# chaofengc/FeMaSR

Hardware: AMD Instinct MI355X
Metric: SR output megapixels/sec at x4 (128->512) (higher is better)
Workload: dtype f32 (1x1 convs / nn.Linear: every fp32 operand split EXACTLY into three bf16 terms, six partial products, fp32 accumulation on the bf16 matrix pipe - closer to fp64 than the fp32 fmaf chain, bit-identical to the CPU oracle)

## Files before the change

femasr_amd/_lib.py:

```python
import ctypes
import os

_HERE = os.path.dirname(os.path.abspath(__file__))
SO_PATH = os.path.join(_HERE, 'csrc', 'libfemasr_hip.so')

c_int, c_i64, c_f32 = ctypes.c_int, ctypes.c_int64, ctypes.c_float
vp, szt = ctypes.c_void_p, ctypes.c_size_t


class FemasrError(RuntimeError):
    pass


MAX_CODEBOOKS = 3


class Config(ctypes.Structure):
    _fields_ = ([(n, ctypes.c_int32) for n in ('in_channel', 'gt_resolution', 'lq_stage', 'scale_factor', 'use_quantize',
                                               'use_residual', 'n_codebooks')] +
                [(n, ctypes.c_int32 * MAX_CODEBOOKS) for n in ('codebook_scale', 'n_e', 'e_dim')] +
                [('device', ctypes.c_int32)])


class ConvArgs(ctypes.Structure):
# ... 107 lines not shown
    'femasr_niqe_plane_offsets': (c_int, [c_int, c_int, c_int, c_int, ctypes.POINTER(szt * 4)]),
    'femasr_niqe_features': (c_int, [vp, vp, c_int, c_int, c_int, c_int, vp, vp, vp, vp, c_int, vp, vp, c_int, vp, vp, vp, szt]),
    'femasr_color_fix_workspace_bytes': (c_int, [c_int, c_int, c_int, c_int, c_int, c_int, ctypes.POINTER(szt)]),
    'femasr_color_fix': (c_int, [vp, vp, vp, c_int, c_int, c_int, c_int, c_int, c_int, c_int, vp, vp, c_int, vp, vp, c_int, vp, vp, szt]),
    'femasr_color_fix_u8': (c_int, [vp, vp, vp, c_int, c_int, c_int, c_int, c_int, c_int, c_int, vp, vp, c_int, vp, vp, c_int, vp, vp, szt]),
    'femasr_dihedral_expand': (c_int, [vp, vp, c_int, c_int, c_int, c_int, vp, vp]),
    'femasr_dihedral_expand_u8': (c_int, [vp, vp, c_int, c_int, c_int, vp, vp]),
    'femasr_dihedral_merge': (c_int, [vp, vp, vp, c_int, c_int, c_int, c_int, vp]),
    'femasr_dihedral_merge_u8': (c_int, [vp, vp, vp, c_int, c_int, c_int, vp]),
    'femasr_png_filter_rgb8': (c_int, [vp, vp, c_int, c_int, c_int, c_int, vp]),
    'femasr_png_filter_u8': (c_int, [vp, vp, c_int, c_int, c_int, c_int, c_int, vp]),
    'femasr_channels_split_u8': (c_int, [vp, vp, c_int, c_int, c_int, c_int, vp, vp]),
    'femasr_channels_merge_u8': (c_int, [vp, vp, vp, vp, c_int, c_int, c_int, c_int, vp, vp, c_int, vp, vp, c_int, vp]),
    'femasr_clock_probe': (c_int, [vp, c_int, vp]),
    'femasr_clock_probe_entries': (c_int, []),
}
DEBUG_SIGNATURES = {
    'femasr_debug_set_wino_limits': (c_int, [vp, c_int, c_int]),
    'femasr_debug_mfma_bf16': (c_int, [vp, vp, vp, vp, c_int, vp]),
    'femasr_gemm_force_config': (c_int, [c_int]),
    'femasr_conv_small_launch_blocks': (c_int, [c_int]),
    'femasr_debug_conv_variant_name': (c_int, [ctypes.POINTER(ConvArgs), ctypes.c_char_p, c_int]),
    'femasr_debug_weight_image_bytes': (c_int, [vp, c_int, ctypes.POINTER(szt)]),
}

_lib = None


def load():
    global _lib
    if _lib is not None:
        return _lib
    if not os.path.exists(SO_PATH):
        raise FemasrError(
            f'{SO_PATH} not found: the HIP extension is not built. Run `python femasr_amd/csrc/build.py` '
            '(needs hipcc; cross-compiles gfx950 without a GPU). There is no CPU fallback.')
    lib = ctypes.CDLL(SO_PATH)
    lib.femasr_version.restype = c_int
    if lib.femasr_version() != ABI_VERSION:
        raise FemasrError(f'{SO_PATH} reports ABI version {lib.femasr_version()}, this binding is written for {ABI_VERSION} '
                          '(femasr_conv_args layout): rebuild with `python femasr_amd/csrc/build.py --force`')
    for name, (res, args) in list(SIGNATURES.items()) + list(DEBUG_SIGNATURES.items()):
        fn = getattr(lib, name)
        fn.restype = res
        fn.argtypes = args
    _lib = lib
# ... 12 lines not shown
```

femasr_amd/csrc/build.py:

```python
import os
import subprocess
import sys

HERE = os.path.dirname(os.path.abspath(__file__))
SOURCES = ['kernels_conv.hip', 'kernels_gemm.hip', 'kernels_gemm_bf16.hip', 'kernels_gemm_f16.hip', 'kernels_vq.hip', 'kernels_norm.hip', 'kernels_attn.hip', 'kernels_layout.hip', 'kernels_probe.hip', 'conv_forms.hip', 'kernels_wino.hip', 'kernels_wino_up2.hip', 'kernels_conv_bf16.hip', 'kernels_conv_f16.hip', 'model.hip', 'lpips.hip', 'psnr_ssim.hip', 'niqe.hip', 'colorfix.hip', 'ensemble.hip', 'png_filter.hip', 'channels.hip']
HEADERS = ['common.h', 'conv_common.h', 'halo_mma.h', 'wino_common.h', 'gemm_common.h', 'detmath.h', 'pixel.h', '../../include/femasr_hip.h', '../../include/femasr_hip_debug.h']
SO = os.path.join(HERE, 'libfemasr_hip.so')
FLAGS = ['--offload-arch=gfx950', '-O3', '-std=c++17', '-fPIC', '-ffp-contract=off',
         '-fhip-fp32-correctly-rounded-divide-sqrt', '-Wno-unused-result']


def _stale(target, deps):
    if not os.path.exists(target):
        return True
    t = os.path.getmtime(target)
    return any(os.path.getmtime(d) > t for d in deps)


def build(force=False, verbose=True, gate='fail'):
    hipcc = os.environ.get('HIPCC', '/opt/rocm/bin/hipcc')
    hdrs = [os.path.join(HERE, h) for h in HEADERS]
    objs, jobs = [], []
    for src in SOURCES:
        s = os.path.join(HERE, src)
        o = os.path.join(HERE, src.replace('.hip', '.o'))
        if force or _stale(o, [s] + hdrs):
            cmd = [hipcc] + FLAGS + ['-c', s, '-o', o]
            if verbose:
                print(' '.join(cmd), flush=True)
# ... 33 lines not shown
```

femasr_amd/csrc/common.h:

```cpp
#pragma once
#include <hip/hip_runtime.h>
#include <stdint.h>
#include <stddef.h>
#include "../../include/femasr_hip_debug.h"

int femasr_set_error(int code, const char *fmt, ...);
#define FEMASR_CHECK_HIP(expr)                                                            \
    do {                                                                                  \
        hipError_t _e = (expr);                                                           \
        if (_e != hipSuccess)                                                             \
            return femasr_set_error(FEMASR_ERR_HIP, "%s failed: %s (%s:%d)", #expr,       \
                                    hipGetErrorString(_e), __FILE__, __LINE__);           \
    } while (0)
#define FEMASR_REQUIRE(cond, ...)                                                         \
    do {                                                                                  \
        if (!(cond)) return femasr_set_error(FEMASR_ERR_INVALID, __VA_ARGS__);            \
    } while (0)

inline int femasr_allow_dynamic_lds(const void *kern, unsigned long long *devs, size_t bytes)
{
    int dev = 0;
    FEMASR_CHECK_HIP(hipGetDevice(&dev));
    if (dev < 0 || dev >= 64 || !((__atomic_load_n(devs, __ATOMIC_ACQUIRE) >> dev) & 1ull)) {
        FEMASR_CHECK_HIP(hipFuncSetAttribute(kern, hipFuncAttributeMaxDynamicSharedMemorySize, (int)bytes));
        if (dev >= 0 && dev < 64) __atomic_fetch_or(devs, 1ull << dev, __ATOMIC_RELEASE);
    }
    return FEMASR_OK;
}
#define FEMASR_CHECK(expr) do { const int _rc = (expr); if (_rc != FEMASR_OK) return _rc; } while (0)

inline unsigned grid_for(size_t total)
{
    const size_t g = (total + 255) / 256;
    return (unsigned)(g < 1 ? 1 : (g > 4096 ? 4096 : g));
}

namespace {
__device__ __forceinline__ float4 ld4(const float *p) { return *reinterpret_cast<const float4 *>(p); }
__device__ __forceinline__ int clampi(int v, int lo, int hi) { return v < lo ? lo : (v > hi ? hi : v); }
}

struct conv_vq_epilogue {
    const float *zz;
    const float *ee;
    float *part;
    int nblk;
};
int femasr_conv2d_launch(hipStream_t s, const femasr_conv_args *a, const conv_vq_epilogue *vq,
                         int *variant_out, double *flops_out);
int femasr_conv2d_pick_variant(const femasr_conv_args *a);
int femasr_conv_variant_count();
const char *femasr_conv_variant_name(int v);
bool femasr_conv_halo_eligible(const femasr_conv_args *a);
inline bool femasr_gn_fusable(int cout) { const int cg = cout / 32; return cout % 32 == 0 && cg >= 1 && cg <= 32 && (cg & (cg - 1)) == 0; }

inline size_t femasr_compact_weight_floats(int O, int I, int kh, int kw)
{
    return (O <= 4 && kh == 3 && kw == 3 && (I % 32) == 0) ? (size_t)I * 9 * 4 : 0;
}

bool femasr_gemm_eligible(const femasr_conv_args *a);
int femasr_gemm_launch(hipStream_t s, const femasr_conv_args *a, const conv_vq_epilogue *vq, int *variant_out, double *flops_out);
// ... 72 lines not shown
```

femasr_amd/csrc/conv_common.h:

```cpp
#pragma once
#include "common.h"

namespace {

struct ConvParams {
    const float *in, *w, *bias, *pro_a, *pro_b, *pro_c, *res1, *res2;
    const float *w_wino;
    const float *w_up2;
    float *out;
    const float *vq_zz, *vq_ee;
    float *vq_part;
    int vq_nblk;
    double *gn_part;
    int B, H, W, Cin, Cout, ksz, stride, pad, up2, act, Ho, Wo;
    int M, K, nchunks, taps, MB, NB, NT32;
    int tilesX, tilesY;
    int kperm;
};

constexpr int BK = 32;
constexpr int ALD = BK + 1;

typedef __attribute__((address_space(1))) const float *gcptr_f32;
typedef __attribute__((address_space(1))) float *gptr_f32;
// ... 26 lines not shown
    *reinterpret_cast<__attribute__((address_space(1))) f32x4_t *>(a + byteoff) = v;
}
constexpr int TPITCH = 36;
constexpr int TSCRATCH = 32 * TPITCH;
constexpr int HALO_EPI_OFF = 2048;

typedef _Float16 f16x2 __attribute__((ext_vector_type(2)));
__device__ __forceinline__ unsigned pack_f16(float x0, float x1)
{
    x0 = __builtin_fminf(__builtin_fmaxf(x0, -65504.f), 65504.f);
    x1 = __builtin_fminf(__builtin_fmaxf(x1, -65504.f), 65504.f);
    const f16x2 h = {(_Float16)x0, (_Float16)x1};
    return __builtin_bit_cast(unsigned, h);
}

__device__ __forceinline__ float f4get(const float4 &v, int i) { return i == 0 ? v.x : (i == 1 ? v.y : (i == 2 ? v.z : v.w)); }

__device__ __forceinline__ int wtile(int n0, int t, int nt32)
{
    const int idx = (n0 >> 5) + t;
    return idx < nt32 ? idx : nt32 - 1;
}

__device__ __forceinline__ int xcd_remap(int bid, int nblk)
{
    const int q = nblk >> 3, r = nblk & 7, xcd = bid & 7, within = bid >> 3;
    return (xcd < r ? xcd * (q + 1) : r * (q + 1) + (xcd - r) * q) + within;
}

struct HaloVariant {
    const char *name;
    int bn, threads;
    void (*kern)(const ConvParams, const uint4 *, double *);
    size_t lds;
    unsigned long long attr_devs;
};

template <int N>
int halo_variant_launch(hipStream_t s, const femasr_conv_args *a, const char *who, HaloVariant (&table)[N], const void *image,
                        bool (*shape_ok)(const femasr_conv_args *), int (*pick)(const femasr_conv_args *), int *variant_out, double *flops_out)
{
    FEMASR_REQUIRE(a && a->in && a->bias && a->out && image && shape_ok(a), "%s: not eligible", who);
    const int Hv = a->up2 ? 2 * a->H : a->H, Wv = a->up2 ? 2 * a->W : a->W;
    FEMASR_REQUIRE(Hv == a->Ho && Wv == a->Wo, "%s: Ho/Wo mismatch", who);
    if (a->prologue == FEMASR_PRO_GN_SILU) FEMASR_REQUIRE(a->pro_a && a->pro_b, "%s: GN prologue needs a,b", who);
    ConvParams p{};
    p.in = a->in; p.bias = a->bias; p.pro_a = a->pro_a; p.pro_b = a->pro_b; p.res1 = a->res1; p.res2 = a->res2; p.out = a->out;
    p.B = a->B; p.H = a->H; p.W = a->W; p.Cin = a->Cin; p.Cout = a->Cout; p.ksz = 3; p.stride = 1; p.pad = 1; p.up2 = a->up2;
    p.Ho = Hv; p.Wo = Wv; p.NT32 = (a->Cout + 31) / 32;
    const int vi = pick(a);
    HaloVariant &v = table[vi];
    p.tilesX = (p.Wo + 15) / 16;
// ... 18 lines not shown
```

femasr_amd/csrc/kernels_attn.hip:

```cpp
#include "common.h"
#include "detmath.h"

namespace {

constexpr int ATT_HD = 32, ATT_N = 64;
typedef float att_f32x16 __attribute__((ext_vector_type(16)));

template <int UNITS>
__global__ __launch_bounds__(64, 2) void window_attention_reg_kernel(const float *__restrict__ qkv, int B, int H, int W, int C,
                                                                     int heads, int shift, const float *__restrict__ table,
                                                                     float *__restrict__ out, int total)
{
    __shared__ float Ts[UNITS][232];
    const int lane = threadIdx.x, c = lane & 31, hf = lane >> 5;
    const int nwx = W >> 3, nwy = H >> 3;
    struct Unit { int h, wx, wy, n; };
    auto unit_of = [&](int bid) {
        Unit g;
        g.h = bid % heads;
        bid /= heads;
        g.wx = bid % nwx;
        bid /= nwx;
        g.wy = bid % nwy;
        g.n = bid / nwy;
        return g;
    };
    Unit gs[UNITS];
    bool has[UNITS];
#pragma unroll
    for (int u = 0; u < UNITS; ++u) {
        const int bid = (int)blockIdx.x * UNITS + u;
        has[u] = bid < total;
        gs[u] = unit_of(has[u] ? bid : total - 1);
        for (int i = lane; i < 225; i += 64) Ts[u][i] = table[i * heads + gs[u].h];
    }
    const float scale = 0.17677669529663687f;
    auto rowtok = [&](const Unit &g, int iy) { int y = g.wy * 8 + iy + shift; if (y >= H) y -= H; return y * W; };
    auto coltok = [&](const Unit &g, int ix) { int x = g.wx * 8 + ix + shift; if (x >= W) x -= W; return x; };
    auto qb = [&](const Unit &g) { return qkv + (size_t)g.n * H * W * 3 * C + g.h * ATT_HD; };

    float ak[2][16], bq[2][16];
    auto load_qk = [&](const Unit &g) {
        const float *qbase = qb(g);
#pragma unroll
        for (int tI = 0; tI < 2; ++tI) {
            const int w = 32 * tI + c;
            const unsigned tok = (unsigned)(rowtok(g, w >> 3) + coltok(g, w & 7));
            const float *kp = qbase + tok * (unsigned)(3 * C) + C, *qp = qbase + tok * (unsigned)(3 * C);
#pragma unroll
            for (int d4 = 0; d4 < 8; ++d4) {
                const float4 kv = ld4(kp + 4 * d4), qv = ld4(qp + 4 * d4);
                ak[tI][2 * d4] = hf ? kv.y : kv.x;
                ak[tI][2 * d4 + 1] = hf ? kv.w : kv.z;
                bq[tI][2 * d4] = (hf ? qv.y : qv.x) * scale;
                bq[tI][2 * d4 + 1] = (hf ? qv.w : qv.z) * scale;
            }
        }
    };
    load_qk(gs[0]);
#pragma unroll
    for (int u = 0; u < UNITS; ++u) {
        if (!has[u]) break;
        const Unit g = gs[u];
        const float *qbase = qb(g);
        float *obase = out + (size_t)g.n * H * W * C + g.h * ATT_HD;
        const bool masked = shift > 0 && (g.wy == nwy - 1 || g.wx == nwx - 1);
        att_f32x16 sc[2][2];
#pragma unroll
        for (int tj = 0; tj < 2; ++tj)
#pragma unroll
            for (int ti = 0; ti < 2; ++ti)
#pragma unroll
                for (int r = 0; r < 16; ++r) sc[tj][ti][r] = 0.f;
#pragma unroll
        for (int st = 0; st < 16; ++st)
#pragma unroll
            for (int tj = 0; tj < 2; ++tj)
#pragma unroll
                for (int ti = 0; ti < 2; ++ti) sc[tj][ti] = __builtin_amdgcn_mfma_f32_32x32x2f32(ak[tj][st], bq[ti][st], sc[tj][ti], 0, 0, 0);

        float vf[2][16];
        {
            const float *vb = qbase + 2 * C + c;
            unsigned cto[4];
#pragma unroll
            for (int e = 0; e < 4; ++e) cto[e] = (unsigned)coltok(g, e + 4 * hf) * (unsigned)(3 * C);
#pragma unroll
            for (int tj = 0; tj < 2; ++tj)
#pragma unroll
                for (int r = 0; r < 16; ++r) {
                    const unsigned ro = (unsigned)__builtin_amdgcn_readfirstlane(rowtok(g, (r >> 2) + 4 * tj)) * (unsigned)(3 * C);
                    vf[tj][r] = vb[ro + cto[r & 3]];
                }
        }
        if (u + 1 < UNITS && has[u + 1 < UNITS ? u + 1 : u]) load_qk(gs[u + 1 < UNITS ? u + 1 : u]);
#pragma unroll
        for (int ti = 0; ti < 2; ++ti) {
            const int i = 32 * ti + c, iy = i >> 3, ix = i & 7;
            const int tb = (iy + 7) * 15 + ix + 7 - 4 * hf;
            unsigned rowdiff = 0, coldiff = 0;
            if (masked) {
                const int ysi = g.wy * 8 + iy, xsi = g.wx * 8 + ix;
                const int ryi = ysi < H - 8 ? 0 : (ysi < H - shift ? 1 : 2), rxi = xsi < W - 8 ? 0 : (xsi < W - shift ? 1 : 2);
#pragma unroll
                for (int q = 0; q < 8; ++q) {
                    const int ysj = g.wy * 8 + q, xsj = g.wx * 8 + q;
                    const int ryj = ysj < H - 8 ? 0 : (ysj < H - shift ? 1 : 2), rxj = xsj < W - 8 ? 0 : (xsj < W - shift ? 1 : 2);
                    rowdiff |= (ryj != ryi ? 1u : 0u) << q;
                    coldiff |= (rxj != rxi ? 1u : 0u) << q;
                }
                coldiff >>= 4 * hf;
            }
            float m = -INFINITY;
#pragma unroll
            for (int tj = 0; tj < 2; ++tj)
#pragma unroll
                for (int r = 0; r < 16; ++r) {
                    const int jy = (r >> 2) + 4 * tj, jxl = r & 3;
                    float a1 = sc[tj][ti][r] + Ts[u][tb - 15 * jy - jxl];
                    if (masked) a1 = a1 + ((((rowdiff >> jy) | (coldiff >> jxl)) & 1u) ? -100.0f : 0.0f);
                    sc[tj][ti][r] = a1;
                    m = a1 > m ? a1 : m;
                }
            {
                const float mo = __shfl_xor(m, 32, 64);
                m = mo > m ? mo : m;
            }
            float part = 0.f;
#pragma unroll
            for (int tj = 0; tj < 2; ++tj)
#pragma unroll
                for (int r = 0; r < 16; r += 2) {
                    const det_f32x2 e = det_expf2(det_f32x2{sc[tj][ti][r] - m, sc[tj][ti][r + 1] - m});
                    sc[tj][ti][r] = e[0];
                    sc[tj][ti][r + 1] = e[1];
                    part = part + e[0];
                    part = part + e[1];
                }
            const float other = __shfl_xor(part, 32, 64);
            const float rinv = 1.0f / (hf ? other + part : part + other);
#pragma unroll
            for (int tj = 0; tj < 2; ++tj) sc[tj][ti] = sc[tj][ti] * rinv;
        }

        att_f32x16 oc[2];
#pragma unroll
        for (int ti = 0; ti < 2; ++ti)
#pragma unroll
            for (int r = 0; r < 16; ++r) oc[ti][r] = 0.f;
#pragma unroll
        for (int tj = 0; tj < 2; ++tj)
#pragma unroll
            for (int r = 0; r < 16; ++r)
#pragma unroll
                for (int ti = 0; ti < 2; ++ti) oc[ti] = __builtin_amdgcn_mfma_f32_32x32x2f32(sc[tj][ti][r], vf[tj][r], oc[ti], 0, 0, 0);

        {
            float *ob = obase + c;
            unsigned cto[4];
#pragma unroll
            for (int e = 0; e < 4; ++e) cto[e] = (unsigned)coltok(g, e + 4 * hf) * (unsigned)C;
#pragma unroll
            for (int ti = 0; ti < 2; ++ti)
#pragma unroll
                for (int r = 0; r < 16; ++r) {
                    const unsigned ro = (unsigned)__builtin_amdgcn_readfirstlane(rowtok(g, (r >> 2) + 4 * ti)) * (unsigned)C;
                    ob[ro + cto[r & 3]] = oc[ti][r];
                }
        }
    }
}

}

extern "C" {

int femasr_window_attention(void *stream, const float *qkv, int B, int H, int W, int C, int heads, int shift,
                            const float *table, float *out)
{
    FEMASR_REQUIRE(qkv && table && out && B > 0, "window_attention: bad args");
    FEMASR_REQUIRE(H % 8 == 0 && W % 8 == 0 && H >= 8 && W >= 8, "window_attention: H,W must be multiples of 8 (%d,%d)", H, W);
    FEMASR_REQUIRE(heads > 0 && heads <= 8 && C == heads * ATT_HD, "window_attention: head_dim must be 32, at most 8 heads (C=%d heads=%d)", C, heads);
    FEMASR_REQUIRE(shift >= 0 && shift < 8, "window_attention: bad shift %d", shift);
    FEMASR_REQUIRE((size_t)H * W * 3 * C < ((size_t)1 << 30), "window_attention: image too large for 32-bit offsets");
    const size_t total = (size_t)B * (H / 8) * (W / 8) * heads;
    FEMASR_REQUIRE(total < ((size_t)1 << 31), "window_attention: too many (window, head) units");
    hipLaunchKernelGGL(window_attention_reg_kernel<1>, dim3((unsigned)total), dim3(64), 0, (hipStream_t)stream, qkv, B, H, W, C, heads, shift, table,
                       out, (int)total);
    FEMASR_CHECK_HIP(hipGetLastError());
    return FEMASR_OK;
}

}
```

femasr_amd/csrc/model.hip:

```cpp
#include <assert.h>
#include <stdarg.h>
#include <stdio.h>
#include <stdlib.h>
#include <string.h>

#include <algorithm>
#include <array>
#include <map>
#include <string>
#include <vector>

#include "common.h"

static thread_local char g_err[1024] = "";

int femasr_set_error(int code, const char *fmt, ...)
{
    va_list ap;
    va_start(ap, fmt);
    vsnprintf(g_err, sizeof(g_err), fmt, ap);
    va_end(ap);
    return code;
}

namespace {

struct DeviceGuard {
    int prev = -1;
    bool ok = true;
    explicit DeviceGuard(int dev)
    {
        if (hipGetDevice(&prev) != hipSuccess) prev = -1;
        if (prev != dev) ok = hipSetDevice(dev) == hipSuccess;
    }
    ~DeviceGuard() { if (prev >= 0) (void)hipSetDevice(prev); }
// ... 6 lines not shown
    case 128: return 128;
    case 256: return 64;
    case 512: return 32;
    default: return -1;
    }
}

int ilog2(int v)
{
    int r = 0;
    while ((1 << (r + 1)) <= v) ++r;
    return r;
}

enum WKind { W_CONV, W_LINEAR, W_VEC, W_TABLE, W_CODEBOOK };

struct WSpec {
    std::string key;
    WKind kind;
    int64_t shape[4];
    int ndim;
    void *image[CONV_FORM_COUNT] = {};
    float *up2w = nullptr;
    float *dev() const { return (float *)image[CONV_DIRECT]; }
    int ksz() const { return kind == W_CONV ? (int)shape[2] : 1; }
    bool up2 = false;
    int stride = 1;
    bool set = false;
    size_t numel() const { size_t n = 1; for (int i = 0; i < ndim; ++i) n *= (size_t)shape[i]; return n; }
};

bool behind_every_lookup(const femasr_config &cfg, int encode_depth, int last_quant_stage, const std::string &k)
{
    const bool dec = k.rfind("decoder_group.", 0) == 0, aq = k.rfind("after_quant_group.", 0) == 0, oc = k.rfind("out_conv", 0) == 0;
    if (cfg.n_codebooks == 1) {
        if (dec || aq || oc) return true;
        const std::string pre = "multiscale_encoder.blocks.";
        return cfg.lq_stage && k.rfind(pre, 0) == 0 && atoi(k.c_str() + pre.size()) > encode_depth;
    }
    if (oc) return true;
    if (aq) return atoi(k.c_str() + 18) == cfg.n_codebooks - 1;
    if (dec) return atoi(k.c_str() + 14) >= last_quant_stage;
    return false;
}

struct T {
    float *p = nullptr;
    int B = 0, H = 0, W = 0, C = 0;
    double *gn_part = nullptr;
    int gn_tiles = 0;
    size_t numel() const { return (size_t)B * H * W * C; }
};

struct Arena {
    char *base = nullptr;
    size_t cap = 0, peak = 0;
    bool dry = true;
    std::map<size_t, size_t> free_;
    std::map<size_t, size_t> used_;
    void reset(void *b, size_t c, bool d)
    {
        base = d ? (char *)4096 : (char *)b; cap = c; dry = d; peak = 0;
        free_.clear(); used_.clear();
        free_[0] = d ? ((size_t)1 << 60) : c;
    }
    void *alloc(size_t bytes)
// ... 38 lines not shown
};

}

struct femasr_handle {
    femasr_config cfg;
    int scale = 1, max_depth = 0, encode_depth = 0;
    int last_quant_stage = 0;
    std::vector<WSpec> specs;
    std::map<std::string, int> index;
    float *cbT[FEMASR_MAX_CODEBOOKS] = {nullptr, nullptr, nullptr}, *ee[FEMASR_MAX_CODEBOOKS] = {nullptr, nullptr, nullptr};
    void *vq_aux[FEMASR_MAX_CODEBOOKS] = {nullptr, nullptr, nullptr};
    bool finalized = false;
    unsigned decoder_seen = ((1u << FEMASR_DECODER_MATH_COUNT) - 1) & ~(1u << FEMASR_DECODER_MATH_FP16);
    unsigned linear_seen = ((1u << FEMASR_LINEAR_MATH_COUNT) - 1) & ~(1u << FEMASR_LINEAR_MATH_FP16);
    bool prof = false;
    std::vector<ProfRec> recs;
    std::vector<hipEvent_t> pool;
    size_t pool_used = 0;
    std::vector<double> acc_ms, acc_flops, acc_bytes;
    std::vector<int64_t> acc_n;
    std::vector<std::string> slot_names;
    ConvModes modes;
    int nsub = 1;
    std::vector<hipStream_t> sub_streams;
    std::vector<hipEvent_t> sub_done;
    hipEvent_t ev_fork = nullptr;
    std::map<std::array<int, 4>, std::vector<size_t>> plans;
};

namespace {

enum { SLOT_GN = 0, SLOT_LN, SLOT_ATTN, SLOT_VQ, SLOT_LAYOUT, SLOT_SMALL_COUNT };
const char *kSmallNames[SLOT_SMALL_COUNT] = {"gn_moments", "layernorm", "window_attention", "vq(codebook lookup)",
                                             "pad/crop/gather layout"};

struct Scope {
    femasr_handle *h;
    ProfRec rec{};
    bool on;
    hipStream_t st;
    Scope(femasr_handle *hh, hipStream_t stream, bool dry, int slot, double flops, double bytes)
        : h(hh), on(hh->prof && !dry), st(stream)
    {
        if (!on) return;
        auto get = [&]() {
// ... 314 lines not shown
        release(u);
        if (free_x) release(x);
        return y;
    }

    T swin_block(const T &y, int B, int H, int W, const std::string &bp, int shift)
    {
        const int rows = B * H * W, C = 256;
        auto ln = [&](const T &t, const std::string &np) {
            T o = alloc_t(1, rows, 1, C);
            if (rc || dry()) return o;
            Scope sc(h, s(), dry(), SLOT_LN, 0.0, (double)t.numel() * 8.0);
            const int r = femasr_layernorm(s(), t.p, rows, C, Wt(np + ".weight"), Wt(np + ".bias"), 1e-5f, o.p);
            if (r && !rc) rc = r;
            return o;
        };
        T n1 = ln(y, bp + ".norm1");
        ConvOpt oq; oq.ksz = 1; oq.pad = 0;
        T qkv = conv(n1, bp + ".attn.qkv", 3 * C, oq);
        release(n1);
        T att = alloc_t(1, rows, 1, C);
        if (!rc && !dry()) {
            Scope sc(h, s(), dry(), SLOT_ATTN, 4.0 * (double)rows * 64.0 * C, (double)rows * C * 16.0);
            const int r = femasr_window_attention(s(), qkv.p, B, H, W, C, 8, shift, Wt(bp + ".attn.relative_position_bias_table"), att.p);
            if (r && !rc) rc = r;
        }
        release(qkv);
        ConvOpt op; op.ksz = 1; op.pad = 0; op.res1 = y.p;
        T y1 = conv(att, bp + ".attn.proj", C, op);
        release(att);
        T n2 = ln(y1, bp + ".norm2");
        ConvOpt o1; o1.ksz = 1; o1.pad = 0; o1.act = FEMASR_ACT_GELU;
        T hdn = conv(n2, bp + ".mlp.fc1", 4 * C, o1);
        release(n2);
        ConvOpt o2; o2.ksz = 1; o2.pad = 0; o2.res1 = y1.p;
        T y2 = conv(hdn, bp + ".mlp.fc2", C, o2);
        release(hdn);
        release(y1);
        return y2;
    }

    T swin_layers(T x, const std::string &sp)
    {
        const int B = x.B, H = x.H, W = x.W, C = x.C;
        for (int r = 0; r < 4; ++r) {
            const std::string rp = sp + ".swin_blks." + std::to_string(r);
            T y; y.p = x.p; y.B = 1; y.H = B * H * W; y.W = 1; y.C = C;
// ... 285 lines not shown
    }
    DeviceGuard guard(cfg->device);
    if (!guard.ok) { delete h; return femasr_set_error(FEMASR_ERR_HIP, "hipSetDevice(%d) failed", cfg->device); }
    const int rc = build_specs(h);
    if (rc) { delete h; return rc; }
    for (int i = 0; i < SLOT_SMALL_COUNT; ++i) h->slot_names.push_back(kSmallNames[i]);
    for (int f = 0; f < CONV_FORM_COUNT; ++f) {
        const ConvFormDesc &d = femasr_conv_form_desc(f);
        assert(d.form == f);
        for (int v = 0; v < d.variant_count(); ++v) h->slot_names.push_back(d.variant_name(v));
    }
    const size_t nslots = h->slot_names.size();
    h->acc_ms.assign(nslots, 0.0); h->acc_flops.assign(nslots, 0.0); h->acc_bytes.assign(nslots, 0.0); h->acc_n.assign(nslots, 0);
    *out = h;
    return FEMASR_OK;
}

void femasr_destroy(femasr_handle *h)
{
    if (!h) return;
    for (auto &w : h->specs) {
        for (void *p : w.image) if (p) (void)hipFree(p);
        if (w.up2w) (void)hipFree(w.up2w);
    }
    for (int q = 0; q < FEMASR_MAX_CODEBOOKS; ++q) {
        if (h->cbT[q]) (void)hipFree(h->cbT[q]);
        if (h->ee[q]) (void)hipFree(h->ee[q]);
        if (h->vq_aux[q]) (void)hipFree(h->vq_aux[q]);
    }
    for (auto e : h->pool) (void)hipEventDestroy(e);
    for (auto e : h->sub_done) (void)hipEventDestroy(e);
    for (auto st : h->sub_streams) (void)hipStreamDestroy(st);
    if (h->ev_fork) (void)hipEventDestroy(h->ev_fork);
    delete h;
}

int femasr_num_weights(const femasr_handle *h) { return h ? (int)h->specs.size() : 0; }

int femasr_weight_info(const femasr_handle *h, int i, const char **key, int64_t shape[4], int *ndim)
{
    FEMASR_REQUIRE(h && i >= 0 && i < (int)h->specs.size(), "weight_info: bad index");
    const WSpec &w = h->specs[i];
    if (key) *key = w.key.c_str();
    if (shape) for (int k = 0; k < 4; ++k) shape[k] = k < w.ndim ? w.shape[k] : 1;
    if (ndim) *ndim = w.ndim;
    return FEMASR_OK;
}

int femasr_set_weight(femasr_handle *h, const char *key, const float *dev_ptr, const int64_t *shape, int ndim)
{
    FEMASR_REQUIRE(h && key && dev_ptr && shape, "set_weight: null argument");
    const std::string k(key);
    if (k.size() > 24 && (k.rfind(".relative_position_index") == k.size() - 24)) return FEMASR_OK;
    if (k.size() > 10 && (k.rfind(".attn_mask") == k.size() - 10)) return FEMASR_OK;
    auto it = h->index.find(k);
    if (it == h->index.end()) return femasr_set_error(FEMASR_ERR_WEIGHT, "set_weight: unknown key '%s'", key);
    DeviceGuard guard(h->cfg.device);
    FEMASR_REQUIRE(guard.ok, "set_weight: hipSetDevice(%d) failed", h->cfg.device);
    WSpec &w = h->specs[it->second];
    bool same = (ndim == w.ndim);
    for (int i = 0; same && i < ndim; ++i) same = (shape[i] == w.shape[i]);
    if (!same) return femasr_set_error(FEMASR_ERR_WEIGHT, "set_weight: shape mismatch for '%s'", key);
    if (w.kind != W_CONV && w.kind != W_LINEAR) {
        if (!w.dev()) FEMASR_CHECK_HIP(hipMalloc(&w.image[CONV_DIRECT], w.numel() * sizeof(float)));
        FEMASR_CHECK_HIP(hipMemcpyAsync(w.dev(), dev_ptr, w.numel() * sizeof(float), hipMemcpyDeviceToDevice, nullptr));
    } else {
        const int O = (int)w.shape[0], I = (int)w.shape[1];
        const std::array<bool, CONV_FORM_COUNT> can = layer_forms(h, w);
        for (int f = 0; f < CONV_FORM_COUNT; ++f) {
            if (!can[f]) continue;
            const ConvFormDesc &d = femasr_conv_form_desc(f);
            if (!w.image[f]) FEMASR_CHECK_HIP(hipMalloc(&w.image[f], d.image_bytes(O, I, w.ksz())));
            FEMASR_CHECK(d.repack(dev_ptr, O, I, w.ksz(), w.image[f]));
        }
        if (w.up2 && femasr_up2_weight_floats(O, I)) {
            if (!w.up2w) FEMASR_CHECK_HIP(hipMalloc((void **)&w.up2w, femasr_up2_weight_floats(O, I) * sizeof(float)));
            FEMASR_CHECK(femasr_repack_oihw_up2(nullptr, dev_ptr, O, I, w.up2w));
        }
    }
    FEMASR_CHECK_HIP(hipStreamSynchronize(nullptr));
    w.set = true;
    h->finalized = false;
    return FEMASR_OK;
}

int femasr_finalize_weights(femasr_handle *h)
{
    FEMASR_REQUIRE(h, "finalize: null handle");
// ... 223 lines not shown
int femasr_debug_set_wino_limits(femasr_handle *h, int log2_total, int log2_image)
{
    FEMASR_REQUIRE(h && log2_total >= 0 && log2_total <= FEMASR_WINO_LOG2_TOTAL && log2_image >= 0 && log2_image <= FEMASR_WINO_LOG2_IMAGE,
                   "debug_set_wino_limits: exponents are 0 (default) or up to %d / %d", FEMASR_WINO_LOG2_TOTAL, FEMASR_WINO_LOG2_IMAGE);
    h->modes.wino_log2_total = log2_total ? log2_total : FEMASR_WINO_LOG2_TOTAL;
    h->modes.wino_log2_image = log2_image ? log2_image : FEMASR_WINO_LOG2_IMAGE;
    h->plans.clear();
    return FEMASR_OK;
}

int femasr_set_linear_math(femasr_handle *h, int mode)
{
    FEMASR_REQUIRE(h && mode >= 0 && mode < FEMASR_LINEAR_MATH_COUNT, "set_linear_math: mode must be 0 (fp32 MFMA chain), 1 (bf16 three-term split) or 2 (fp16, one pass)");
    if (!(h->linear_seen >> mode & 1)) {
        h->linear_seen |= 1u << mode;
        const int rc = build_missing_images(h, "set_linear_math");
        if (rc) { h->linear_seen &= ~(1u << mode); return rc; }
    }
    if (h->modes.linear_math != mode) h->plans.clear();
    h->modes.linear_math = mode;
    return FEMASR_OK;
}

int femasr_debug_weight_image_bytes(const femasr_handle *h, int form, size_t *bytes)
{
    FEMASR_REQUIRE(h && bytes && form >= 0 && form < CONV_FORM_COUNT, "debug_weight_image_bytes: bad args");
    *bytes = 0;
    for (const auto &w : h->specs)
        if ((w.kind == W_CONV || w.kind == W_LINEAR) && w.image[form])
            *bytes += femasr_conv_form_desc(form).image_bytes((int)w.shape[0], (int)w.shape[1], w.ksz());
    return FEMASR_OK;
}

int femasr_profile_enable(femasr_handle *h, int on)
{
    FEMASR_REQUIRE(h, "null handle");
    h->prof = on != 0;
    return FEMASR_OK;
}

static int profile_drain(femasr_handle *h)
{
    for (auto &r : h->recs) {
        FEMASR_CHECK_HIP(hipEventSynchronize(r.e1));
        float ms = 0.f;
        FEMASR_CHECK_HIP(hipEventElapsedTime(&ms, r.e0, r.e1));
// ... 42 lines not shown
```

include/femasr_hip_debug.h:

```cpp
#ifndef FEMASR_HIP_DEBUG_H
#define FEMASR_HIP_DEBUG_H
#include "femasr_hip.h"
#ifdef __cplusplus
extern "C" {
#endif

int femasr_debug_set_wino_limits(femasr_handle *h, int log2_total, int log2_image);

int femasr_debug_mfma_bf16(void *stream, const uint16_t *a, const uint16_t *b, const float *c, int n, float *d);

int femasr_gemm_force_config(int cfg);
int femasr_conv_small_launch_blocks(int blocks);

int femasr_debug_conv_variant_name(const femasr_conv_args *a, char *name, int cap);

int femasr_debug_weight_image_bytes(const femasr_handle *h, int form, size_t *bytes);

#ifdef __cplusplus
}
#endif
#endif
```

Measured before the change: 68.05.

## Restructure window attention loads: head-major bias table, vector Q/K loads, prefetch V

Repacks the relative-position bias table at weight-load time into a head-major padded image so each block loads its head's table with one float4 per lane instead of strided scalar loads. Q/K rows are now loaded as 4 contiguous float4s per half-wave and redistributed with permlane32_swap rather than 8 float4s with lane-dependent selects. V loading is split so part is issued before the score MFMAs and the rest overlaps them, and blocks are remapped across XCDs. This adds a second table copy per layer and a debug path that keeps the raw-table kernel.

Measured after the change: 68.38 (median of 6 runs). No clear change (+0.5%).

```diff
diff --git a/femasr_amd/_lib.py b/femasr_amd/_lib.py
--- a/femasr_amd/_lib.py
+++ b/femasr_amd/_lib.py
@@ -153,6 +153,8 @@
     'femasr_conv_small_launch_blocks': (c_int, [c_int]),
     'femasr_debug_conv_variant_name': (c_int, [ctypes.POINTER(ConvArgs), ctypes.c_char_p, c_int]),
     'femasr_debug_weight_image_bytes': (c_int, [vp, c_int, ctypes.POINTER(szt)]),
+    'femasr_debug_attn_raw_table': (c_int, [vp, c_int]),
+    'femasr_debug_window_attention_image': (c_int, [vp, vp, c_int, c_int, c_int, c_int, c_int, c_int, vp, vp, vp]),
 }
 
 _lib = None
diff --git a/femasr_amd/csrc/attn_kernel.h b/femasr_amd/csrc/attn_kernel.h
--- /dev/null
+++ b/femasr_amd/csrc/attn_kernel.h
@@ -0,0 +1,237 @@
+#pragma once
+#include "common.h"
+#include "detmath.h"
+
+namespace {
+
+constexpr int ATT_HD = 32, ATT_N = 64;
+constexpr int ATT_TABLE_PITCH = 232;
+typedef float att_f32x16 __attribute__((ext_vector_type(16)));
+
+template <int UNITS, bool HM>
+__global__ __launch_bounds__(64, 2) void window_attention_reg_kernel(const float *__restrict__ qkv, int B, int H, int W, int C,
+                                                                     int heads, int shift, const float *__restrict__ table,
+                                                                     float *__restrict__ out, int total)
+{
+    __shared__ __attribute__((aligned(16))) float Ts[UNITS][ATT_TABLE_PITCH];
+    const int lane = threadIdx.x, c = lane & 31, hf = lane >> 5;
+    const int nwx = W >> 3, nwy = H >> 3;
+    struct Unit { int h, wx, wy, n; };
+    auto unit_of = [&](int bid) {
+        Unit g;
+        g.h = bid % heads;
+        bid /= heads;
+        g.wx = bid % nwx;
+        bid /= nwx;
+        g.wy = bid % nwy;
+        g.n = bid / nwy;
+        return g;
+    };
+    Unit gs[UNITS];
+    bool has[UNITS];
+    const int blk = xcd_remap((int)blockIdx.x, (int)gridDim.x);
+#pragma unroll
+    for (int u = 0; u < UNITS; ++u) {
+        const int bid = blk * UNITS + u;
+        has[u] = bid < total;
+        gs[u] = unit_of(has[u] ? bid : total - 1);
+    }
+    float4 tv[UNITS];
+    auto load_table = [&](int u) {
+        if (HM) {
+            if (lane < ATT_TABLE_PITCH / 4) tv[u] = ld4(table + gs[u].h * ATT_TABLE_PITCH + 4 * lane);
+        } else {
+            tv[u].x = table[lane * heads + gs[u].h];
+            tv[u].y = table[(lane + 64) * heads + gs[u].h];
+            tv[u].z = table[(lane + 128) * heads + gs[u].h];
+            if (lane + 192 < 225) tv[u].w = table[(lane + 192) * heads + gs[u].h];
+        }
+    };
+    auto store_table = [&](int u) {
+        if (HM) {
+            if (lane < ATT_TABLE_PITCH / 4) *reinterpret_cast<float4 *>(&Ts[u][4 * lane]) = tv[u];
+        } else {
+            Ts[u][lane] = tv[u].x;
+            Ts[u][lane + 64] = tv[u].y;
+            Ts[u][lane + 128] = tv[u].z;
+            if (lane + 192 < 225) Ts[u][lane + 192] = tv[u].w;
+        }
+    };
+    const float scale = 0.17677669529663687f;
+    auto rowtok = [&](const Unit &g, int iy) { int y = g.wy * 8 + iy + shift; if (y >= H) y -= H; return y * W; };
+    auto coltok = [&](const Unit &g, int ix) { int x = g.wx * 8 + ix + shift; if (x >= W) x -= W; return x; };
+    auto qb = [&](const Unit &g) { return qkv + (size_t)g.n * H * W * 3 * C + g.h * ATT_HD; };
+
+    float ak[2][16], bq[2][16];
+    float4 kr[2][4], qr[2][4];
+    auto load_qk = [&](const Unit &g) {
+        const float *qbase = qb(g);
+#pragma unroll
+        for (int tI = 0; tI < 2; ++tI) {
+            const int w = 32 * tI + c;
+            const unsigned tok = (unsigned)(rowtok(g, w >> 3) + coltok(g, w & 7));
+            const float *kp = qbase + tok * (unsigned)(3 * C) + C, *qp = qbase + tok * (unsigned)(3 * C);
+#pragma unroll
+            for (int d4 = 0; d4 < 4; ++d4) {
+                kr[tI][d4] = ld4(kp + 16 * hf + 4 * d4);
+                qr[tI][d4] = ld4(qp + 16 * hf + 4 * d4);
+            }
+        }
+    };
+    auto trade_qk = [&]() {
+#pragma unroll
+        for (int tI = 0; tI < 2; ++tI)
+#pragma unroll
+            for (int k = 0; k < 8; ++k) {
+                const float4 kv = kr[tI][k >> 1], qv = qr[tI][k >> 1];
+                const auto ks = __builtin_amdgcn_permlane32_swap(__builtin_bit_cast(unsigned, (k & 1) ? kv.z : kv.x),
+                                                                 __builtin_bit_cast(unsigned, (k & 1) ? kv.w : kv.y), false, false);
+                const auto qs = __builtin_amdgcn_permlane32_swap(__builtin_bit_cast(unsigned, (k & 1) ? qv.z : qv.x),
+                                                                 __builtin_bit_cast(unsigned, (k & 1) ? qv.w : qv.y), false, false);
+                ak[tI][k] = __builtin_bit_cast(float, (unsigned)ks[0]);
+                ak[tI][8 + k] = __builtin_bit_cast(float, (unsigned)ks[1]);
+                bq[tI][k] = __builtin_bit_cast(float, (unsigned)qs[0]) * scale;
+                bq[tI][8 + k] = __builtin_bit_cast(float, (unsigned)qs[1]) * scale;
+            }
+    };
+    float vf[2][16];
+    auto load_v = [&](const Unit &g, int t0, int t1) {
+        const float *vb = qb(g) + 2 * C + c;
+        unsigned cto[4];
+#pragma unroll
+        for (int e = 0; e < 4; ++e) cto[e] = (unsigned)coltok(g, e + 4 * hf) * (unsigned)(3 * C);
+#pragma unroll
+        for (int tj = t0; tj < t1; ++tj)
+#pragma unroll
+            for (int r = 0; r < 16; ++r) {
+                const unsigned ro = (unsigned)__builtin_amdgcn_readfirstlane(rowtok(g, (r >> 2) + 4 * tj)) * (unsigned)(3 * C);
+                vf[tj][r] = vb[ro + cto[r & 3]];
+            }
+    };
+    load_qk(gs[0]);
+#pragma unroll
+    for (int u = 0; u < UNITS; ++u) load_table(u);
+    load_v(gs[0], 0, 1);
+#pragma unroll
+    for (int u = 0; u < UNITS; ++u) {
+        if (!has[u]) break;
+        const Unit g = gs[u];
+        float *obase = out + (size_t)g.n * H * W * C + g.h * ATT_HD;
+        const bool masked = shift > 0 && (g.wy == nwy - 1 || g.wx == nwx - 1);
+        if (u == 0) {
+            __builtin_amdgcn_sched_barrier(0);
+#pragma unroll
+            for (int v = 0; v < UNITS; ++v) store_table(v);
+        }
+        trade_qk();
+        att_f32x16 sc[2][2];
+#pragma unroll
+        for (int tj = 0; tj < 2; ++tj)
+#pragma unroll
+            for (int ti = 0; ti < 2; ++ti)
+#pragma unroll
+                for (int r = 0; r < 16; ++r) sc[tj][ti][r] = 0.f;
+#pragma unroll
+        for (int st = 0; st < 16; ++st)
+#pragma unroll
+            for (int tj = 0; tj < 2; ++tj)
+#pragma unroll
+                for (int ti = 0; ti < 2; ++ti) sc[tj][ti] = __builtin_amdgcn_mfma_f32_32x32x2f32(ak[tj][st], bq[ti][st], sc[tj][ti], 0, 0, 0);
+
+        load_v(g, u == 0 ? 1 : 0, 2);
+        if (u + 1 < UNITS && has[u + 1 < UNITS ? u + 1 : u]) load_qk(gs[u + 1 < UNITS ? u + 1 : u]);
+#pragma unroll
+        for (int ti = 0; ti < 2; ++ti) {
+            const int i = 32 * ti + c, iy = i >> 3, ix = i & 7;
+            const int tb = (iy + 7) * 15 + ix + 7 - 4 * hf;
+            unsigned rowdiff = 0, coldiff = 0;
+            if (masked) {
+                const int ysi = g.wy * 8 + iy, xsi = g.wx * 8 + ix;
+                const int ryi = ysi < H - 8 ? 0 : (ysi < H - shift ? 1 : 2), rxi = xsi < W - 8 ? 0 : (xsi < W - shift ? 1 : 2);
+#pragma unroll
+                for (int q = 0; q < 8; ++q) {
+                    const int ysj = g.wy * 8 + q, xsj = g.wx * 8 + q;
+                    const int ryj = ysj < H - 8 ? 0 : (ysj < H - shift ? 1 : 2), rxj = xsj < W - 8 ? 0 : (xsj < W - shift ? 1 : 2);
+                    rowdiff |= (ryj != ryi ? 1u : 0u) << q;
+                    coldiff |= (rxj != rxi ? 1u : 0u) << q;
+                }
+                coldiff >>= 4 * hf;
+            }
+            float m = -INFINITY;
+#pragma unroll
+            for (int tj = 0; tj < 2; ++tj)
+#pragma unroll
+                for (int r = 0; r < 16; ++r) {
+                    const int jy = (r >> 2) + 4 * tj, jxl = r & 3;
+                    float a1 = sc[tj][ti][r] + Ts[u][tb - 15 * jy - jxl];
+                    if (masked) a1 = a1 + ((((rowdiff >> jy) | (coldiff >> jxl)) & 1u) ? -100.0f : 0.0f);
+                    sc[tj][ti][r] = a1;
+                    m = a1 > m ? a1 : m;
+                }
+            {
+                const float mo = __shfl_xor(m, 32, 64);
+                m = mo > m ? mo : m;
+            }
+            float part = 0.f;
+#pragma unroll
+            for (int tj = 0; tj < 2; ++tj)
+#pragma unroll
+                for (int r = 0; r < 16; r += 2) {
+                    const det_f32x2 e = det_expf2(det_f32x2{sc[tj][ti][r] - m, sc[tj][ti][r + 1] - m});
+                    sc[tj][ti][r] = e[0];
+                    sc[tj][ti][r + 1] = e[1];
+                    part = part + e[0];
+                    part = part + e[1];
+                }
+            const float other = __shfl_xor(part, 32, 64);
+            const float rinv = 1.0f / (hf ? other + part : part + other);
+#pragma unroll
+            for (int tj = 0; tj < 2; ++tj) sc[tj][ti] = sc[tj][ti] * rinv;
+        }
+
+        att_f32x16 oc[2];
+#pragma unroll
+        for (int ti = 0; ti < 2; ++ti)
+#pragma unroll
+            for (int r = 0; r < 16; ++r) oc[ti][r] = 0.f;
+#pragma unroll
+        for (int tj = 0; tj < 2; ++tj)
+#pragma unroll
+            for (int r = 0; r < 16; ++r)
+#pragma unroll
+                for (int ti = 0; ti < 2; ++ti) oc[ti] = __builtin_amdgcn_mfma_f32_32x32x2f32(sc[tj][ti][r], vf[tj][r], oc[ti], 0, 0, 0);
+
+        {
+            float *ob = obase + c;
+            unsigned cto[4];
+#pragma unroll
+            for (int e = 0; e < 4; ++e) cto[e] = (unsigned)coltok(g, e + 4 * hf) * (unsigned)C;
+#pragma unroll
+            for (int ti = 0; ti < 2; ++ti)
+#pragma unroll
+                for (int r = 0; r < 16; ++r) {
+                    const unsigned ro = (unsigned)__builtin_amdgcn_readfirstlane(rowtok(g, (r >> 2) + 4 * ti)) * (unsigned)C;
+                    ob[ro + cto[r & 3]] = oc[ti][r];
+                }
+        }
+    }
+}
+
+template <bool HM>
+int window_attention_launch(hipStream_t stream, const float *qkv, int B, int H, int W, int C, int heads, int shift, const float *table,
+                            float *out)
+{
+    FEMASR_REQUIRE(qkv && table && out && B > 0, "window_attention: bad args");
+    FEMASR_REQUIRE(H % 8 == 0 && W % 8 == 0 && H >= 8 && W >= 8, "window_attention: H,W must be multiples of 8 (%d,%d)", H, W);
+    FEMASR_REQUIRE(heads > 0 && heads <= 8 && C == heads * ATT_HD, "window_attention: head_dim must be 32, at most 8 heads (C=%d heads=%d)", C, heads);
+    FEMASR_REQUIRE(shift >= 0 && shift < 8, "window_attention: bad shift %d", shift);
+    FEMASR_REQUIRE((size_t)H * W * 3 * C < ((size_t)1 << 30), "window_attention: image too large for 32-bit offsets");
+    const size_t total = (size_t)B * (H / 8) * (W / 8) * heads;
+    FEMASR_REQUIRE(total < ((size_t)1 << 31), "window_attention: too many (window, head) units");
+    hipLaunchKernelGGL((window_attention_reg_kernel<1, HM>), dim3((unsigned)total), dim3(64), 0, stream, qkv, B, H, W, C, heads, shift, table,
+                       out, (int)total);
+    FEMASR_CHECK_HIP(hipGetLastError());
+    return FEMASR_OK;
+}
+
+}
diff --git a/femasr_amd/csrc/build.py b/femasr_amd/csrc/build.py
--- a/femasr_amd/csrc/build.py
+++ b/femasr_amd/csrc/build.py
@@ -4,7 +4,7 @@
 
 HERE = os.path.dirname(os.path.abspath(__file__))
 SOURCES = ['kernels_conv.hip', 'kernels_gemm.hip', 'kernels_gemm_bf16.hip', 'kernels_gemm_f16.hip', 'kernels_vq.hip', 'kernels_norm.hip', 'kernels_attn.hip', 'kernels_layout.hip', 'kernels_probe.hip', 'conv_forms.hip', 'kernels_wino.hip', 'kernels_wino_up2.hip', 'kernels_conv_bf16.hip', 'kernels_conv_f16.hip', 'model.hip', 'lpips.hip', 'psnr_ssim.hip', 'niqe.hip', 'colorfix.hip', 'ensemble.hip', 'png_filter.hip', 'channels.hip']
-HEADERS = ['common.h', 'conv_common.h', 'halo_mma.h', 'wino_common.h', 'gemm_common.h', 'detmath.h', 'pixel.h', '../../include/femasr_hip.h', '../../include/femasr_hip_debug.h']
+HEADERS = ['common.h', 'attn_kernel.h', 'conv_common.h', 'halo_mma.h', 'wino_common.h', 'gemm_common.h', 'detmath.h', 'pixel.h', '../../include/femasr_hip.h', '../../include/femasr_hip_debug.h']
 SO = os.path.join(HERE, 'libfemasr_hip.so')
 FLAGS = ['--offload-arch=gfx950', '-O3', '-std=c++17', '-fPIC', '-ffp-contract=off',
          '-fhip-fp32-correctly-rounded-divide-sqrt', '-Wno-unused-result']
diff --git a/femasr_amd/csrc/common.h b/femasr_amd/csrc/common.h
--- a/femasr_amd/csrc/common.h
+++ b/femasr_amd/csrc/common.h
@@ -38,6 +38,11 @@
 namespace {
 __device__ __forceinline__ float4 ld4(const float *p) { return *reinterpret_cast<const float4 *>(p); }
 __device__ __forceinline__ int clampi(int v, int lo, int hi) { return v < lo ? lo : (v > hi ? hi : v); }
+__device__ __forceinline__ int xcd_remap(int bid, int nblk)
+{
+    const int q = nblk >> 3, r = nblk & 7, xcd = bid & 7, within = bid >> 3;
+    return (xcd < r ? xcd * (q + 1) : r * (q + 1) + (xcd - r) * q) + within;
+}
 }
 
 struct conv_vq_epilogue {
diff --git a/femasr_amd/csrc/conv_common.h b/femasr_amd/csrc/conv_common.h
--- a/femasr_amd/csrc/conv_common.h
+++ b/femasr_amd/csrc/conv_common.h
@@ -72,12 +72,6 @@
     return idx < nt32 ? idx : nt32 - 1;
 }
 
-__device__ __forceinline__ int xcd_remap(int bid, int nblk)
-{
-    const int q = nblk >> 3, r = nblk & 7, xcd = bid & 7, within = bid >> 3;
-    return (xcd < r ? xcd * (q + 1) : r * (q + 1) + (xcd - r) * q) + within;
-}
-
 struct HaloVariant {
     const char *name;
     int bn, threads;
diff --git a/femasr_amd/csrc/kernels_attn.hip b/femasr_amd/csrc/kernels_attn.hip
--- a/femasr_amd/csrc/kernels_attn.hip
+++ b/femasr_amd/csrc/kernels_attn.hip
@@ -1,194 +1,11 @@
-#include "common.h"
-#include "detmath.h"
-
-namespace {
-
-constexpr int ATT_HD = 32, ATT_N = 64;
-typedef float att_f32x16 __attribute__((ext_vector_type(16)));
-
-template <int UNITS>
-__global__ __launch_bounds__(64, 2) void window_attention_reg_kernel(const float *__restrict__ qkv, int B, int H, int W, int C,
-                                                                     int heads, int shift, const float *__restrict__ table,
-                                                                     float *__restrict__ out, int total)
-{
-    __shared__ float Ts[UNITS][232];
-    const int lane = threadIdx.x, c = lane & 31, hf = lane >> 5;
-    const int nwx = W >> 3, nwy = H >> 3;
-    struct Unit { int h, wx, wy, n; };
-    auto unit_of = [&](int bid) {
-        Unit g;
-        g.h = bid % heads;
-        bid /= heads;
-        g.wx = bid % nwx;
-        bid /= nwx;
-        g.wy = bid % nwy;
-        g.n = bid / nwy;
-        return g;
-    };
-    Unit gs[UNITS];
-    bool has[UNITS];
-#pragma unroll
-    for (int u = 0; u < UNITS; ++u) {
-        const int bid = (int)blockIdx.x * UNITS + u;
-        has[u] = bid < total;
-        gs[u] = unit_of(has[u] ? bid : total - 1);
-        for (int i = lane; i < 225; i += 64) Ts[u][i] = table[i * heads + gs[u].h];
-    }
-    const float scale = 0.17677669529663687f;
-    auto rowtok = [&](const Unit &g, int iy) { int y = g.wy * 8 + iy + shift; if (y >= H) y -= H; return y * W; };
-    auto coltok = [&](const Unit &g, int ix) { int x = g.wx * 8 + ix + shift; if (x >= W) x -= W; return x; };
-    auto qb = [&](const Unit &g) { return qkv + (size_t)g.n * H * W * 3 * C + g.h * ATT_HD; };
-
-    float ak[2][16], bq[2][16];
-    auto load_qk = [&](const Unit &g) {
-        const float *qbase = qb(g);
-#pragma unroll
-        for (int tI = 0; tI < 2; ++tI) {
-            const int w = 32 * tI + c;
-            const unsigned tok = (unsigned)(rowtok(g, w >> 3) + coltok(g, w & 7));
-            const float *kp = qbase + tok * (unsigned)(3 * C) + C, *qp = qbase + tok * (unsigned)(3 * C);
-#pragma unroll
-            for (int d4 = 0; d4 < 8; ++d4) {
-                const float4 kv = ld4(kp + 4 * d4), qv = ld4(qp + 4 * d4);
-                ak[tI][2 * d4] = hf ? kv.y : kv.x;
-                ak[tI][2 * d4 + 1] = hf ? kv.w : kv.z;
-                bq[tI][2 * d4] = (hf ? qv.y : qv.x) * scale;
-                bq[tI][2 * d4 + 1] = (hf ? qv.w : qv.z) * scale;
-            }
-        }
-    };
-    load_qk(gs[0]);
-#pragma unroll
-    for (int u = 0; u < UNITS; ++u) {
-        if (!has[u]) break;
-        const Unit g = gs[u];
-        const float *qbase = qb(g);
-        float *obase = out + (size_t)g.n * H * W * C + g.h * ATT_HD;
-        const bool masked = shift > 0 && (g.wy == nwy - 1 || g.wx == nwx - 1);
-        att_f32x16 sc[2][2];
-#pragma unroll
-        for (int tj = 0; tj < 2; ++tj)
-#pragma unroll
-            for (int ti = 0; ti < 2; ++ti)
-#pragma unroll
-                for (int r = 0; r < 16; ++r) sc[tj][ti][r] = 0.f;
-#pragma unroll
-        for (int st = 0; st < 16; ++st)
-#pragma unroll
-            for (int tj = 0; tj < 2; ++tj)
-#pragma unroll
-                for (int ti = 0; ti < 2; ++ti) sc[tj][ti] = __builtin_amdgcn_mfma_f32_32x32x2f32(ak[tj][st], bq[ti][st], sc[tj][ti], 0, 0, 0);
-
-        float vf[2][16];
-        {
-            const float *vb = qbase + 2 * C + c;
-            unsigned cto[4];
-#pragma unroll
-            for (int e = 0; e < 4; ++e) cto[e] = (unsigned)coltok(g, e + 4 * hf) * (unsigned)(3 * C);
-#pragma unroll
-            for (int tj = 0; tj < 2; ++tj)
-#pragma unroll
-                for (int r = 0; r < 16; ++r) {
-                    const unsigned ro = (unsigned)__builtin_amdgcn_readfirstlane(rowtok(g, (r >> 2) + 4 * tj)) * (unsigned)(3 * C);
-                    vf[tj][r] = vb[ro + cto[r & 3]];
-                }
-        }
-        if (u + 1 < UNITS && has[u + 1 < UNITS ? u + 1 : u]) load_qk(gs[u + 1 < UNITS ? u + 1 : u]);
-#pragma unroll
-        for (int ti = 0; ti < 2; ++ti) {
-            const int i = 32 * ti + c, iy = i >> 3, ix = i & 7;
-            const int tb = (iy + 7) * 15 + ix + 7 - 4 * hf;
-            unsigned rowdiff = 0, coldiff = 0;
-            if (masked) {
-                const int ysi = g.wy * 8 + iy, xsi = g.wx * 8 + ix;
-                const int ryi = ysi < H - 8 ? 0 : (ysi < H - shift ? 1 : 2), rxi = xsi < W - 8 ? 0 : (xsi < W - shift ? 1 : 2);
-#pragma unroll
-                for (int q = 0; q < 8; ++q) {
-                    const int ysj = g.wy * 8 + q, xsj = g.wx * 8 + q;
-                    const int ryj = ysj < H - 8 ? 0 : (ysj < H - shift ? 1 : 2), rxj = xsj < W - 8 ? 0 : (xsj < W - shift ? 1 : 2);
-                    rowdiff |= (ryj != ryi ? 1u : 0u) << q;
-                    coldiff |= (rxj != rxi ? 1u : 0u) << q;
-                }
-                coldiff >>= 4 * hf;
-            }
-            float m = -INFINITY;
-#pragma unroll
-            for (int tj = 0; tj < 2; ++tj)
-#pragma unroll
-                for (int r = 0; r < 16; ++r) {
-                    const int jy = (r >> 2) + 4 * tj, jxl = r & 3;
-                    float a1 = sc[tj][ti][r] + Ts[u][tb - 15 * jy - jxl];
-                    if (masked) a1 = a1 + ((((rowdiff >> jy) | (coldiff >> jxl)) & 1u) ? -100.0f : 0.0f);
-                    sc[tj][ti][r] = a1;
-                    m = a1 > m ? a1 : m;
-                }
-            {
-                const float mo = __shfl_xor(m, 32, 64);
-                m = mo > m ? mo : m;
-            }
-            float part = 0.f;
-#pragma unroll
-            for (int tj = 0; tj < 2; ++tj)
-#pragma unroll
-                for (int r = 0; r < 16; r += 2) {
-                    const det_f32x2 e = det_expf2(det_f32x2{sc[tj][ti][r] - m, sc[tj][ti][r + 1] - m});
-                    sc[tj][ti][r] = e[0];
-                    sc[tj][ti][r + 1] = e[1];
-                    part = part + e[0];
-                    part = part + e[1];
-                }
-            const float other = __shfl_xor(part, 32, 64);
-            const float rinv = 1.0f / (hf ? other + part : part + other);
-#pragma unroll
-            for (int tj = 0; tj < 2; ++tj) sc[tj][ti] = sc[tj][ti] * rinv;
-        }
-
-        att_f32x16 oc[2];
-#pragma unroll
-        for (int ti = 0; ti < 2; ++ti)
-#pragma unroll
-            for (int r = 0; r < 16; ++r) oc[ti][r] = 0.f;
-#pragma unroll
-        for (int tj = 0; tj < 2; ++tj)
-#pragma unroll
-            for (int r = 0; r < 16; ++r)
-#pragma unroll
-                for (int ti = 0; ti < 2; ++ti) oc[ti] = __builtin_amdgcn_mfma_f32_32x32x2f32(sc[tj][ti][r], vf[tj][r], oc[ti], 0, 0, 0);
-
-        {
-            float *ob = obase + c;
-            unsigned cto[4];
-#pragma unroll
-            for (int e = 0; e < 4; ++e) cto[e] = (unsigned)coltok(g, e + 4 * hf) * (unsigned)C;
-#pragma unroll
-            for (int ti = 0; ti < 2; ++ti)
-#pragma unroll
-                for (int r = 0; r < 16; ++r) {
-                    const unsigned ro = (unsigned)__builtin_amdgcn_readfirstlane(rowtok(g, (r >> 2) + 4 * ti)) * (unsigned)C;
-                    ob[ro + cto[r & 3]] = oc[ti][r];
-                }
-        }
-    }
-}
-
-}
+#include "attn_kernel.h"
 
 extern "C" {
 
 int femasr_window_attention(void *stream, const float *qkv, int B, int H, int W, int C, int heads, int shift,
                             const float *table, float *out)
 {
-    FEMASR_REQUIRE(qkv && table && out && B > 0, "window_attention: bad args");
-    FEMASR_REQUIRE(H % 8 == 0 && W % 8 == 0 && H >= 8 && W >= 8, "window_attention: H,W must be multiples of 8 (%d,%d)", H, W);
-    FEMASR_REQUIRE(heads > 0 && heads <= 8 && C == heads * ATT_HD, "window_attention: head_dim must be 32, at most 8 heads (C=%d heads=%d)", C, heads);
-    FEMASR_REQUIRE(shift >= 0 && shift < 8, "window_attention: bad shift %d", shift);
-    FEMASR_REQUIRE((size_t)H * W * 3 * C < ((size_t)1 << 30), "window_attention: image too large for 32-bit offsets");
-    const size_t total = (size_t)B * (H / 8) * (W / 8) * heads;
-    FEMASR_REQUIRE(total < ((size_t)1 << 31), "window_attention: too many (window, head) units");
-    hipLaunchKernelGGL(window_attention_reg_kernel<1>, dim3((unsigned)total), dim3(64), 0, (hipStream_t)stream, qkv, B, H, W, C, heads, shift, table,
-                       out, (int)total);
-    FEMASR_CHECK_HIP(hipGetLastError());
-    return FEMASR_OK;
+    return window_attention_launch<false>((hipStream_t)stream, qkv, B, H, W, C, heads, shift, table, out);
 }
 
 }
diff --git a/femasr_amd/csrc/model.hip b/femasr_amd/csrc/model.hip
--- a/femasr_amd/csrc/model.hip
+++ b/femasr_amd/csrc/model.hip
@@ -10,7 +10,7 @@
 #include <string>
 #include <vector>
 
-#include "common.h"
+#include "attn_kernel.h"
 
 static thread_local char g_err[1024] = "";
 
@@ -63,6 +63,7 @@
     int ndim;
     void *image[CONV_FORM_COUNT] = {};
     float *up2w = nullptr;
+    float *table_hm = nullptr;
     float *dev() const { return (float *)image[CONV_DIRECT]; }
     int ksz() const { return kind == W_CONV ? (int)shape[2] : 1; }
     bool up2 = false;
@@ -83,6 +84,22 @@
     if (aq) return atoi(k.c_str() + 18) == cfg.n_codebooks - 1;
     if (dec) return atoi(k.c_str() + 14) >= last_quant_stage;
     return false;
+}
+
+__global__ void attn_table_image_kernel(const float *__restrict__ table, int heads, float *__restrict__ image)
+{
+    const int i = blockIdx.x * blockDim.x + threadIdx.x;
+    if (i >= heads * ATT_TABLE_PITCH) return;
+    const int h = i / ATT_TABLE_PITCH, e = i - h * ATT_TABLE_PITCH;
+    image[i] = e < 225 ? table[e * heads + h] : 0.f;
+}
+
+int attn_table_image(hipStream_t s, const float *table, int heads, float *image)
+{
+    FEMASR_REQUIRE(table && image && heads > 0 && heads <= 8, "attn_table_image: bad args");
+    hipLaunchKernelGGL(attn_table_image_kernel, dim3(grid_for((size_t)heads * ATT_TABLE_PITCH)), dim3(256), 0, s, table, heads, image);
+    FEMASR_CHECK_HIP(hipGetLastError());
+    return FEMASR_OK;
 }
 
 struct T {
@@ -167,6 +184,7 @@
     std::vector<int64_t> acc_n;
     std::vector<std::string> slot_names;
     ConvModes modes;
+    bool attn_raw_table = false;
     int nsub = 1;
     std::vector<hipStream_t> sub_streams;
     std::vector<hipEvent_t> sub_done;
@@ -527,7 +545,10 @@
         T att = alloc_t(1, rows, 1, C);
         if (!rc && !dry()) {
             Scope sc(h, s(), dry(), SLOT_ATTN, 4.0 * (double)rows * 64.0 * C, (double)rows * C * 16.0);
-            const int r = femasr_window_attention(s(), qkv.p, B, H, W, C, 8, shift, Wt(bp + ".attn.relative_position_bias_table"), att.p);
+            const WSpec *tb = spec(bp + ".attn.relative_position_bias_table");
+            const int r = !tb ? rc
+                          : h->attn_raw_table ? femasr_window_attention(s(), qkv.p, B, H, W, C, 8, shift, tb->dev(), att.p)
+                                              : window_attention_launch<true>(s(), qkv.p, B, H, W, C, 8, shift, tb->table_hm, att.p);
             if (r && !rc) rc = r;
         }
         release(qkv);
@@ -859,6 +880,7 @@
     for (auto &w : h->specs) {
         for (void *p : w.image) if (p) (void)hipFree(p);
         if (w.up2w) (void)hipFree(w.up2w);
+        if (w.table_hm) (void)hipFree(w.table_hm);
     }
     for (int q = 0; q < FEMASR_MAX_CODEBOOKS; ++q) {
         if (h->cbT[q]) (void)hipFree(h->cbT[q]);
@@ -901,6 +923,12 @@
     if (w.kind != W_CONV && w.kind != W_LINEAR) {
         if (!w.dev()) FEMASR_CHECK_HIP(hipMalloc(&w.image[CONV_DIRECT], w.numel() * sizeof(float)));
         FEMASR_CHECK_HIP(hipMemcpyAsync(w.dev(), dev_ptr, w.numel() * sizeof(float), hipMemcpyDeviceToDevice, nullptr));
+        if (w.kind == W_TABLE) {
+            const int heads = (int)w.shape[1];
+            FEMASR_REQUIRE(w.shape[0] == 225 && heads > 0 && heads <= 8, "set_weight: '%s' is not a [225][heads <= 8] table", key);
+            if (!w.table_hm) FEMASR_CHECK_HIP(hipMalloc((void **)&w.table_hm, (size_t)heads * ATT_TABLE_PITCH * sizeof(float)));
+            FEMASR_CHECK(attn_table_image(nullptr, dev_ptr, heads, w.table_hm));
+        }
     } else {
         const int O = (int)w.shape[0], I = (int)w.shape[1];
         const std::array<bool, CONV_FORM_COUNT> can = layer_forms(h, w);
@@ -1170,6 +1198,20 @@
     return FEMASR_OK;
 }
 
+int femasr_debug_attn_raw_table(femasr_handle *h, int on)
+{
+    FEMASR_REQUIRE(h, "debug_attn_raw_table: null handle");
+    h->attn_raw_table = on != 0;
+    return FEMASR_OK;
+}
+
+int femasr_debug_window_attention_image(void *stream, const float *qkv, int B, int H, int W, int C, int heads, int shift, const float *table,
+                                        float *image, float *out)
+{
+    FEMASR_CHECK(attn_table_image((hipStream_t)stream, table, heads, image));
+    return window_attention_launch<true>((hipStream_t)stream, qkv, B, H, W, C, heads, shift, image, out);
+}
+
 int femasr_debug_weight_image_bytes(const femasr_handle *h, int form, size_t *bytes)
 {
     FEMASR_REQUIRE(h && bytes && form >= 0 && form < CONV_FORM_COUNT, "debug_weight_image_bytes: bad args");
diff --git a/include/femasr_hip_debug.h b/include/femasr_hip_debug.h
--- a/include/femasr_hip_debug.h
+++ b/include/femasr_hip_debug.h
@@ -16,6 +16,10 @@
 
 int femasr_debug_weight_image_bytes(const femasr_handle *h, int form, size_t *bytes);
 
+int femasr_debug_attn_raw_table(femasr_handle *h, int on);
+int femasr_debug_window_attention_image(void *stream, const float *qkv, int B, int H, int W, int C, int heads, int shift,
+                                        const float *table, float *image, float *out);
+
 #ifdef __cplusplus
 }
 #endif
```
